# mwickert/scikit-dsp-comm

Measured on AMD Instinct MI355X. Metric: complex64 MSamples/s (FIR-1024 tap, 2^26 samples), higher is better.
Workload: dtype c64

## Files before the change

### scikit-dsp-comm_amd/csrc/fir_bank.hip

```cpp
#include "skdsp_internal.hpp"
#include "ols4k_tables.hpp"
#include "tile_walk.hpp"

namespace skdsp {

using namespace ols4k;
typedef float bank_v2f __attribute__((ext_vector_type(2)));

constexpr int64_t kBankTableCap = (int64_t)256 << 20;

struct FirBankHandle : HandleBase {
    int ntaps = 0, nbands = 0, ov = 0, V = 0;
    bool xr = false;
    DevTable<float2> tw, T2;
    DevTable<float4> Hp;
    DevTable<double> g64;
};

struct BankArgs {
    const void *x;
    cf *y;
    int64_t n, row_stride;
    const float2 *tw, *T2;
    const float4 *Hp;
// ... 65 lines not shown
        const float *x = reinterpret_cast<const float *>(A.x);
#pragma unroll 1
        for (int k = 0; k < c.ntaps && k <= m; ++k) {
            const double xv = (double)x[m - k];
            re += c.taps[2 * k] * xv;
            im += c.taps[2 * k + 1] * xv;
        }
    } else {
        careful_fir_point<float, true>(reinterpret_cast<const float *>(A.x), 0, c, 1, 1, m, &re, &im);
    }
    A.y[(size_t)band * A.row_stride + m] = make_float2((float)re, (float)im);
}

template <bool XR> __global__ __launch_bounds__(256, 2) void bank4k_kernel(BankArgs A)
{
    __shared__ cf img[kImgUnits];
    __shared__ cf T2f[kT2Units], T2t[kT2Units];
    __shared__ cf twl[kTwUnits];
    __shared__ unsigned long long noted_word;
    const int t = threadIdx.x;
    if (t == 0) noted_word = 0;
    walk::twiddles_4k(t, A.T2, A.tw, T2f, T2t, twl);
    __syncthreads();
    int64_t step = 0;
    for (int64_t item = blockIdx.x; item < A.items; item += gridDim.x, ++step) {
        const int group = (int)(item / A.ntiles);
        const int64_t tile = item - (int64_t)group * A.ntiles;
        const int b0 = group * A.per;
        const int b1 = b0 + A.per < A.nbands ? b0 + A.per : A.nbands;
        const int64_t out0 = tile * A.V;
        const int64_t in0 = out0 - A.ov;
        cf Z[16];
        float4 hh[8];
        bank_load_H(A, b0, t, hh);
        if (in0 >= 0 && in0 + kN <= A.n) {
            bank_load_interior<XR>(A, in0, t, Z);
        } else {
            bank_load_edge<XR>(A.x, in0, A.n, t, Z);
        }
        fwd_pass1(t, Z, twl, img);
        __syncthreads();
        fwd_pass2(t, T2f, img);
        fwd_pass3(t, img, Z);
        bool poisoned = false;
#pragma unroll 1
        for (int band = b0; band < b1; ++band) {
            cf P[16];
            mul_H(hh, Z, P);
            if (band + 1 < b1) bank_load_H(A, band + 1, t, hh);
            inv_pass3(t, T2t, img, P);
            inv_pass2(t, img);
            __syncthreads();
            inv_pass1(t, twl, img, P);
            __syncthreads();
            poisoned = poisoned || not_finite(P[15]);
            bank_store(A, band, out0, t, P);
        }
        if (__builtin_expect(__any(poisoned), 0)) careful_note(&noted_word, step);
    }
    const unsigned long long noted = careful_noted(&noted_word);
    if (__builtin_expect(noted != 0, 0)) {
        int64_t k = 0;
        for (int64_t item = blockIdx.x; item < A.items; item += gridDim.x, ++k) {
            if (!careful_step_noted(noted, k)) continue;
            const int group = (int)(item / A.ntiles);
            const int64_t out0 = (item - (int64_t)group * A.ntiles) * A.V;
            const int b0 = group * A.per;
            const int b1 = b0 + A.per < A.nbands ? b0 + A.per : A.nbands;
#pragma unroll 1
            for (int band = b0; band < b1; ++band)
#pragma unroll 1
                for (int i = t; i < A.V; i += 256) {
                    if (out0 + i >= A.n) break;
                    bank_careful_point<XR>(A, band, out0 + i);
                }
        }
    }
}

constexpr int kBankFwdCost = 3;
static int bank_bands_per_group(int64_t ntiles, int nbands, int64_t slots)
{
    int best = nbands;
    int64_t best_cost = INT64_MAX;
    for (int g = 1; g <= nbands; ++g) {
        const int per = (nbands + g - 1) / g;
        const int gg = (nbands + per - 1) / per;
// ... 84 lines not shown
```

### scikit-dsp-comm_amd/csrc/fir_dn4k.hip

```cpp
#include "skdsp_internal.hpp"
#include "ols4k_tables.hpp"
#include "tile_walk.hpp"

namespace skdsp {

using namespace ols4k;
typedef float v4f_t __attribute__((ext_vector_type(4)));
typedef float v2f_t __attribute__((ext_vector_type(2)));

struct Dn4kPlan : TilePlan {
    int ov = 0, V = 0;
    DevTable<float2> tw, T2;
    DevTable<float4> Hp;
};

struct Dn4kArgs {
    const void *x;
    void *y;
    int64_t n, n_hist;
    int64_t n_out;
    const float2 *tw, *T2;
    const float4 *Hp;
    int ov, V, a0;
    int M;
// ... 107 lines not shown
{
#pragma unroll 1
    for (int a = a0; a < 16; ++a) {
        const int64_t o = out0 + 256 * (a - a0) + t;
        if (REAL) {
            if (o < n_out) careful_fir_store<float, false>(reinterpret_cast<const float *>(x), n_hist, cf, 1, M, o, reinterpret_cast<float *>(y) + o);
            if (o + V < n_out) careful_fir_store<float, false>(reinterpret_cast<const float *>(x), n_hist, cf, 1, M, o + V, reinterpret_cast<float *>(y) + o + V);
        } else if (o < n_out) {
            careful_fir_store<float, true>(reinterpret_cast<const float *>(x), n_hist, cf, 1, M, o, reinterpret_cast<float *>(y) + 2 * o);
        }
    }
}

template <bool REAL, int MS> __global__ __launch_bounds__(256, 2) void dn4k_kernel(Dn4kArgs A)
{
    __shared__ cf img[kImgUnits];
    __shared__ cf T2f[kT2Units], T2t[kT2Units];
    __shared__ cf twl[kTwUnits];
    __shared__ unsigned long long dn_noted;
    const int t = threadIdx.x;
    if (t == 0) dn_noted = 0;
    walk::twiddles_4k(t, A.T2, A.tw, T2f, T2t, twl);
    __syncthreads();
    int64_t tile = walk::first_tile();
    cf in[MS * 16];
    bool have_in = false;
    for (; tile < A.ntiles; tile += gridDim.x) {
        const bool pre_next = tile + gridDim.x < A.ntiles && dn4k_interior<REAL>(A, tile + gridDim.x);
        if (!have_in) {
            if (dn4k_interior<REAL>(A, tile)) {
                dn4k_load_interior<REAL, MS>(A, tile, 0, t, in);
            } else {
                static_for<0, MS>([&](auto jc) __attribute__((always_inline)) {
                    constexpr int j = decltype(jc)::value;
                    cf e[16];
                    dn4k_load_edge<REAL>(A.x, dn4k_k0<REAL>(A, tile), A.V, A.M, j, A.n_hist, A.n, t, e);
#pragma unroll
                    for (int a = 0; a < 16; ++a) in[16 * j + a] = e[a];
                });
            }
        }
        have_in = pre_next;
        cf acc[16];
        static_for<0, MS>([&](auto jc) __attribute__((always_inline)) {
            constexpr int j = decltype(jc)::value;
            float4 hh[8];
            walk::load_H(A.Hp, j, t, hh);
            cf *Z = in + 16 * j;
            fwd_pass1(t, Z, twl, img);
            __syncthreads();
            fwd_pass2(t, T2f, img, Z);
            fwd_pass3(t, img, Z);
            walk::pin<16>(Z);
            if (j == 0) mul_H(hh, Z, acc); else mac_H(hh, Z, acc);
            walk::pin<16>(acc);
            __syncthreads();
        });
        if (pre_next) dn4k_load_interior<REAL, MS>(A, tile + gridDim.x, 0, t, in);
        inv_pass3(t, T2t, img, acc);
        inv_pass2(t, img);
        __syncthreads();
        inv_pass1(t, twl, img, acc);
        __syncthreads();
        walk::pin<16>(acc);
        if (pre_next) static_for<0, MS>([&](auto jc) __attribute__((always_inline)) { walk::pin<16>(in + 16 * decltype(jc)::value); });
        dn4k_store<REAL>(A, tile, t, acc);
        if (__builtin_expect(__any(not_finite(acc[15].x) | not_finite(acc[15].y)), 0)) careful_note(&dn_noted, (tile - walk::first_tile()) / gridDim.x);
    }
    const unsigned long long noted = careful_noted(&dn_noted);
    if (__builtin_expect(noted != 0, 0)) {
        int64_t k = 0;
        for (int64_t tl = walk::first_tile(); tl < A.ntiles; tl += gridDim.x, ++k)
            if (careful_step_noted(noted, k))
                dn4k_careful_outputs<REAL>(A.x, A.y, A.n_out, A.n_hist, A.cf, A.M, tl * (REAL ? 2 : 1) * (int64_t)A.V, A.V, A.a0, t);
    }
}

bool fir_dn4k_supported(const FirHandle *h, int M)
{
    if (M < 2 || M > 4) return false;
    const int T = dn_taps_per_phase(h->ntaps, M);
    if (T - 1 > 2048) return false;
    return h->dtype == SKDSP_C64 || (h->dtype == SKDSP_F32 && !h->taps_complex);
}

static int dn4k_plan(FirHandle *h, int M, Dn4kPlan **out)
{
    return tile_plan(h->dn4k, M, out, [&](Dn4kPlan &p) {
        tile_overlap(dn_taps_per_phase(h->ntaps, M), 256, kN, &p.ov, &p.V);
        std::vector<float2> tw, T2;
        std::vector<float4> Hp;
        make_tw(tw);
        make_T2(T2);
        make_dn_tables(h->taps_host.data(), h->ntaps, h->taps_complex ? 2 : 1, M, Hp);
        int rc = p.tw.upload(tw);
        if (!rc) rc = p.T2.upload(T2);
        if (!rc) rc = p.Hp.upload(Hp);
// ... 40 lines not shown
```

### scikit-dsp-comm_amd/csrc/fir_ols.hip

```cpp
#include "skdsp_internal.hpp"
#include "ols_tables.hpp"
#include <cstdlib>
#include <cstdio>


namespace skdsp {

using namespace ols;
typedef float v4f_t __attribute__((ext_vector_type(4)));

struct OlsPlan {
    int ntaps = 0;
    int ov = 0;
    int V = 0;
    float4 *T1 = nullptr, *T2 = nullptr, *Hp = nullptr;
};

struct OlsArgs {
    const cf *x;
    cf *y;
    int64_t n, n_hist;
    const float4 *T1, *T2, *Hp;
    int ov, V, a0;
    int keep;
// ... 104 lines not shown
        const int64_t q0 = out0 / A.dec;
        const unsigned r0 = (unsigned)(out0 - q0 * A.dec);
        const unsigned ob = r0 != 0 ? 1u : 0u;
        cf *buf = reinterpret_cast<cf *>(lds);
        int a0 = A.a0;
        asm volatile("" : "+s"(a0));
        __syncthreads();
#pragma unroll
        for (int a = 0; a < 16; ++a) {
            if (a < a0) continue;
#pragma unroll
            for (int e = 0; e < 2; ++e) {
                const unsigned gl = r0 + 512u * (unsigned)(a - a0) + 2u * (unsigned)t + (unsigned)e;
                const unsigned q = (unsigned)(((unsigned long long)gl * A.dec_magic) >> 32);
                if (q * M == gl) buf[q - ob] = v[2 * a + e];
            }
        }
        __syncthreads();
        int64_t oe = q0 + (int64_t)((r0 + (unsigned)A.V + M - 1) / M);
        const int64_t n_out = A.n_keep / A.dec;
        if (oe > n_out) oe = n_out;
        const int cnt = (int)(oe - (q0 + ob));
        cf *yo = A.y + q0 + ob;
        for (int i = t; i < cnt; i += 256) {
            const v2f_t o = {buf[i].x, buf[i].y};
            __builtin_nontemporal_store(o, reinterpret_cast<v2f_t *>(yo + i));
        }
        return;
    }
    if (full) {
        int tt = t;
        asm volatile("" : "+v"(tt));
        float4 *yp = reinterpret_cast<float4 *>(A.y + out0 + 2 * tt);
        auto stores = [&](auto a0c) __attribute__((always_inline)) {
            constexpr int A0 = decltype(a0c)::value;
#pragma unroll
            for (int a = A0; a < 16; ++a) {
                v4f_t nv;
                nv.x = v[2 * a].x; nv.y = v[2 * a].y; nv.z = v[2 * a + 1].x; nv.w = v[2 * a + 1].y;
                __builtin_nontemporal_store(nv, reinterpret_cast<v4f_t *>(yp) + (a - A0) * 256);
            }
        };
        switch (A.a0) {
            case 1: stores(std::integral_constant<int, 1>{}); break;
            case 2: stores(std::integral_constant<int, 2>{}); break;
            case 3: stores(std::integral_constant<int, 3>{}); break;
            case 4: stores(std::integral_constant<int, 4>{}); break;
// ... 286 lines not shown
{
    __shared__ float4 lds[kLdsUnits];
    __shared__ float4 t2lds[2 * kT2Units];
    __shared__ unsigned long long ols_noted;
    if (threadIdx.x == 0) ols_noted = 0;
    constexpr int HS = (DEC && !UP) ? (REAL ? 4 : 5) : 0;
    float4 *T2f = t2lds;
    float4 *T2t = t2lds + kT2Units;
    const int t = threadIdx.x;

    {
        const float4 w = A.T2[t];
        T2f[t] = w;
        T2t[(t & 15) * 16 + (t >> 4)] = w;
    }
    cf tw[16];
#pragma unroll
    for (int k1 = 1; k1 < 16; ++k1) tw[k1] = lo(A.T1[k1 * 256 + t]);
    tw[0] = make_float2(1.f, 0.f);

    __syncthreads();
    int it = 0;
    float4 hh[16];
    int64_t tile = (gridDim.x % 8 == 0) ? (int64_t)(blockIdx.x % 8) * (gridDim.x / 8) + blockIdx.x / 8
                                                                 : (int64_t)blockIdx.x;
    const bool t0_last = A.halo_flag != nullptr;
    auto phys = [&](int64_t w) -> int64_t {
        if (UP) return (int64_t)((unsigned)w / (unsigned)A.up);
        return t0_last ? (w + 1 < A.ntiles ? w + 1 : 0) : w;
    };
    auto phase_of = [&](int64_t w) -> int { return (int)((unsigned)w % (unsigned)A.up); };
    if (!UP) load_H(t, A.Hp, hh);
    cf v[32];
    if (tile < A.ntiles) {
        if (t0_last && phys(tile) == 0) wait_halo(A);
        load_any<REAL, XR>(A, phys(tile), t, v);
    }
    if constexpr (XR) {
#pragma unroll
        for (int i = 0; i < 32; i += 8)
            asm volatile("" ::"v"(v[i].x), "v"(v[i + 1].x), "v"(v[i + 2].x), "v"(v[i + 3].x), "v"(v[i + 4].x), "v"(v[i + 5].x), "v"(v[i + 6].x), "v"(v[i + 7].x));
    } else {
#pragma unroll
    for (int i = 0; i < 32; i += 8)
        asm volatile("" ::"v"(v[i].x), "v"(v[i].y), "v"(v[i + 1].x), "v"(v[i + 1].y), "v"(v[i + 2].x), "v"(v[i + 2].y),
                     "v"(v[i + 3].x), "v"(v[i + 3].y), "v"(v[i + 4].x), "v"(v[i + 4].y), "v"(v[i + 5].x), "v"(v[i + 5].y),
                     "v"(v[i + 6].x), "v"(v[i + 6].y), "v"(v[i + 7].x), "v"(v[i + 7].y));
    }
    for (; tile < A.ntiles; tile += gridDim.x, ++it) {
        if (HS > 0) {
            int tt = t;
            asm volatile("" : "+v"(tt));
#pragma unroll
            for (int j = 16 - HS; j < 16; ++j) hh[j] = vld(reinterpret_cast<const volatile float4 *>(A.Hp) + (unsigned)(j * 256 + tt));
        }
        if (UP) {
            int tt = t;
            asm volatile("" : "+v"(tt));
            const volatile float4 *hp = reinterpret_cast<const volatile float4 *>(A.Hp) + (size_t)phase_of(tile) * 4096;
#pragma unroll
            for (int j = 0; j < 16; ++j) hh[j] = vld(hp + (unsigned)(j * 256 + tt));
        }
        if (REAL) fwd_pass1_real(t, v, tw, lds); else fwd_pass1(t, v, tw, lds);
        __syncthreads();
        cf Z[32];
        fwd_pass23(t, T2f, lds, Z);
        mul_H(hh, Z);
        const int64_t next = tile + gridDim.x;
        cf nx[32];
        __builtin_amdgcn_s_setprio(3);
        if (next < A.ntiles) {
            if (t0_last && phys(next) == 0) wait_halo(A);
            load_any<REAL, XR>(A, phys(next), t, nx);
        }
        __builtin_amdgcn_s_setprio(0);
        inv_pass32(t, T2t, lds, Z);
        __syncthreads();
        inv_pass1(t, tw, lds, v);
        if constexpr (XR) {
#pragma unroll
            for (int i = 0; i < 32; i += 8)
                asm volatile("" ::"v"(nx[i].x), "v"(nx[i + 1].x), "v"(nx[i + 2].x), "v"(nx[i + 3].x), "v"(nx[i + 4].x), "v"(nx[i + 5].x), "v"(nx[i + 6].x), "v"(nx[i + 7].x)
                             : "memory");
        } else {
#pragma unroll
        for (int i = 0; i < 32; i += 8)
            asm volatile("" ::"v"(nx[i].x), "v"(nx[i].y), "v"(nx[i + 1].x), "v"(nx[i + 1].y), "v"(nx[i + 2].x), "v"(nx[i + 2].y),
                         "v"(nx[i + 3].x), "v"(nx[i + 3].y), "v"(nx[i + 4].x), "v"(nx[i + 4].y), "v"(nx[i + 5].x), "v"(nx[i + 5].y),
                         "v"(nx[i + 6].x), "v"(nx[i + 6].y), "v"(nx[i + 7].x), "v"(nx[i + 7].y)
                         : "memory");
        }
        __builtin_amdgcn_s_setprio(3);
        if (UP) {
            if (!DEC && A.up_pitch) {
                OlsArgs B = A;
                B.y = REAL ? reinterpret_cast<cf *>(reinterpret_cast<float *>(A.y) + (int64_t)phase_of(tile) * A.up_pitch) : A.y + (int64_t)phase_of(tile) * A.up_pitch;
                store_any<REAL, false>(B, phys(tile), t, v, lds);
            } else if (REAL) {
                store_tile_real_up<DEC>(A, phys(tile), phase_of(tile), t, v);
            } else {
                store_tile_up<DEC>(A, phys(tile), phase_of(tile), t, v);
            }
        } else {
            store_any<REAL, DEC>(A, phys(tile), t, v, lds);
        }
        __builtin_amdgcn_s_setprio(0);
        if (__builtin_expect(__any(not_finite(v[31].x) | not_finite(v[31].y)), 0)) careful_note(&ols_noted, it);
#pragma unroll
        for (int i = 0; i < 32; ++i) v[i] = nx[i];
#ifdef SK_OLS_KEEP_B3
        __syncthreads();
#else
        if constexpr (REAL || DEC || UP || XR) __syncthreads();
#endif
    }
    const unsigned long long noted = careful_noted(&ols_noted);
    if (__builtin_expect(noted != 0, 0)) {
        int64_t w = (gridDim.x % 8 == 0) ? (int64_t)(blockIdx.x % 8) * (gridDim.x / 8) + blockIdx.x / 8 : (int64_t)blockIdx.x;
        for (int64_t k = 0; w < A.ntiles; w += gridDim.x, ++k)
            if (careful_step_noted(noted, k))
                careful_ols_tile<float, REAL, DEC, UP, XR>(ols_careful_args(A, UP ? phase_of(w) : 0, !(REAL || XR)), phys(w), UP ? phase_of(w) : 0, t);
    }
}


template <bool REAL, int MF>
__global__ __launch_bounds__(256, 2) void ols_fold_kernel(OlsArgs A)
{
    __shared__ float4 lds[kLdsUnits];
    __shared__ float4 t2lds[2 * kT2Units];
    __shared__ unsigned long long ols_noted;
    if (threadIdx.x == 0) ols_noted = 0;
    float4 *T2f = t2lds, *T2t = t2lds + kT2Units;
    const int t = threadIdx.x;
    {
        const float4 w = A.T2[t];
        T2f[t] = w;
        T2t[(t & 15) * 16 + (t >> 4)] = w;
    }
    cf tw[16];
#pragma unroll
    for (int k1 = 1; k1 < 16; ++k1) tw[k1] = lo(A.T1[k1 * 256 + t]);
    tw[0] = make_float2(1.f, 0.f);
    __syncthreads();
    float4 hh[16];
    auto first_tile = [&]() -> int64_t { return (gridDim.x % 8 == 0) ? (int64_t)(blockIdx.x % 8) * (gridDim.x / 8) + blockIdx.x / 8 : (int64_t)blockIdx.x; };
    int64_t tile = first_tile();
    load_H(t, A.Hp, hh);
    cf v[32];
    if (tile < A.ntiles) load_any<REAL, false>(A, tile, t, v);
#pragma unroll
    for (int i = 0; i < 32; i += 8)
        asm volatile("" ::"v"(v[i].x), "v"(v[i].y), "v"(v[i + 1].x), "v"(v[i + 1].y), "v"(v[i + 2].x), "v"(v[i + 2].y),
                     "v"(v[i + 3].x), "v"(v[i + 3].y), "v"(v[i + 4].x), "v"(v[i + 4].y), "v"(v[i + 5].x), "v"(v[i + 5].y),
                     "v"(v[i + 6].x), "v"(v[i + 6].y), "v"(v[i + 7].x), "v"(v[i + 7].y));
    constexpr int LS = MF / 2;
    const int b = t >> 4, q = t & 15;
    const bool active = q % LS == 0;
    const int j0 = (32 / MF) * b + q / LS;
    constexpr int JA = 512 / MF;
    for (int64_t step = 0; tile < A.ntiles; tile += gridDim.x, ++step) {
        if (REAL) fwd_pass1_real(t, v, tw, lds); else fwd_pass1(t, v, tw, lds);
        __syncthreads();
        cf Z[32];
        fwd_pass23(t, T2f, lds, Z);
        mul_H(hh, Z);
        const int64_t next = tile + gridDim.x;
        cf nx[32];
        __builtin_amdgcn_s_setprio(3);
        if (next < A.ntiles) load_any<REAL, false>(A, next, t, nx);
        __builtin_amdgcn_s_setprio(0);
        inv_pass32_fold<MF>(t, T2t, lds, Z);
        __syncthreads();
        cf o[16];
#pragma unroll
        for (int a = 0; a < 16; ++a) o[a] = make_float2(0.f, 0.f);
        inv_pass1_fold<MF>(t, tw, lds, o);
#pragma unroll
        for (int i = 0; i < 32; i += 8)
            asm volatile("" ::"v"(nx[i].x), "v"(nx[i].y), "v"(nx[i + 1].x), "v"(nx[i + 1].y), "v"(nx[i + 2].x), "v"(nx[i + 2].y),
                         "v"(nx[i + 3].x), "v"(nx[i + 3].y), "v"(nx[i + 4].x), "v"(nx[i + 4].y), "v"(nx[i + 5].x), "v"(nx[i + 5].y),
                         "v"(nx[i + 6].x), "v"(nx[i + 6].y), "v"(nx[i + 7].x), "v"(nx[i + 7].y)
                         : "memory");
        __builtin_amdgcn_s_setprio(3);
        if (active) {
            int a0 = A.a0;
            asm volatile("" : "+s"(a0));
            const int Mr = A.dec / MF;
            const int64_t n_out = A.n_keep / A.dec;
            const int VD = A.V / MF;
            const int64_t e0 = (REAL ? 2 * tile : tile) * (int64_t)VD;
            const int64_t q0 = Mr > 1 ? e0 / Mr : e0;
            const unsigned r0 = Mr > 1 ? (unsigned)(e0 - q0 * Mr) : 0u;
// ... 7 lines not shown
                }
            };
#pragma unroll
            for (int a = 0; a < 16; ++a) {
                if (a < a0) continue;
                const unsigned el = (unsigned)(j0 + JA * (a - a0));
                if (REAL) {
                    put(el, o[a].x, reinterpret_cast<float *>(A.y));
                    put(el + (unsigned)VD, o[a].y, reinterpret_cast<float *>(A.y));
                } else {
                    put(el, v2f_t{o[a].x, o[a].y}, reinterpret_cast<v2f_t *>(A.y));
                }
            }
        }
        __builtin_amdgcn_s_setprio(0);
        if (__builtin_expect(__any(active && (not_finite(o[15].x) | not_finite(o[15].y))), 0)) careful_note(&ols_noted, step);
#pragma unroll
        for (int i = 0; i < 32; ++i) v[i] = nx[i];
#ifdef SK_OLS_KEEP_B3
        __syncthreads();
#else
        if constexpr (REAL) __syncthreads();
#endif
    }
    const unsigned long long noted = careful_noted(&ols_noted);
    if (__builtin_expect(noted != 0, 0)) {
        int64_t w = first_tile();
        for (int64_t k = 0; w < A.ntiles; w += gridDim.x, ++k)
            if (careful_step_noted(noted, k)) careful_ols_tile<float, REAL, true, false, false>(ols_careful_args(A, 0, !REAL), w, 0, t);
    }
}


template <bool REAL, int LF>
__device__ __forceinline__ void load_rep(const OlsArgs &A, int64_t tile, int t, cf *in)
{
    constexpr int LS = LF / 2, JA = 512 / LF;
    const int b = t >> 4, q = t & 15;
#pragma unroll
    for (int a = 0; a < 16; ++a) in[a] = make_float2(0.f, 0.f);
    if (q % LS != 0) return;
    const int j0 = (32 / LF) * b + q / LS;
    const int Lr = A.rep_lr;
    const int64_t in0 = (REAL ? 2 * tile : tile) * (int64_t)A.V - A.ov;
    const int64_t e0 = in0 / LF;
    int64_t q0 = e0, r0 = 0;
    if (Lr > 1) {
        q0 = e0 / Lr;
        r0 = e0 - q0 * Lr;
        if (r0 < 0) { r0 += Lr; q0 -= 1; }
    }
    const int VD = A.V / LF;
// ... 37 lines not shown
    }
}

template <bool REAL, int LF>
__global__ __launch_bounds__(256, 2) void ols_rep_kernel(OlsArgs A)
{
    __shared__ float4 lds[kLdsUnits];
    __shared__ float4 t2lds[2 * kT2Units];
    __shared__ unsigned long long ols_noted;
    if (threadIdx.x == 0) ols_noted = 0;
    float4 *T2f = t2lds, *T2t = t2lds + kT2Units;
    const int t = threadIdx.x;
    {
        const float4 w = A.T2[t];
        T2f[t] = w;
        T2t[(t & 15) * 16 + (t >> 4)] = w;
    }
    cf tw[16];
#pragma unroll
    for (int k1 = 1; k1 < 16; ++k1) tw[k1] = lo(A.T1[k1 * 256 + t]);
    tw[0] = make_float2(1.f, 0.f);
    __syncthreads();
    float4 hh[16];
    auto first_tile = [&]() -> int64_t { return (gridDim.x % 8 == 0) ? (int64_t)(blockIdx.x % 8) * (gridDim.x / 8) + blockIdx.x / 8 : (int64_t)blockIdx.x; };
    int64_t tile = first_tile();
    load_H(t, A.Hp, hh);
    cf in[16];
    if (tile < A.ntiles) load_rep<REAL, LF>(A, tile, t, in);
#pragma unroll
    for (int i = 0; i < 16; i += 8)
        asm volatile("" ::"v"(in[i].x), "v"(in[i].y), "v"(in[i + 1].x), "v"(in[i + 1].y), "v"(in[i + 2].x), "v"(in[i + 2].y),
                     "v"(in[i + 3].x), "v"(in[i + 3].y), "v"(in[i + 4].x), "v"(in[i + 4].y), "v"(in[i + 5].x), "v"(in[i + 5].y),
                     "v"(in[i + 6].x), "v"(in[i + 6].y), "v"(in[i + 7].x), "v"(in[i + 7].y));
    for (int64_t step = 0; tile < A.ntiles; tile += gridDim.x, ++step) {
        fwd_pass1_rep<LF>(t, in, tw, lds);
        __syncthreads();
        cf Z[32];
        fwd_pass23_rep<LF>(t, T2f, lds, Z);
        mul_H(hh, Z);
        const int64_t next = tile + gridDim.x;
        cf nx[16];
        __builtin_amdgcn_s_setprio(3);
        if (next < A.ntiles) load_rep<REAL, LF>(A, next, t, nx);
        __builtin_amdgcn_s_setprio(0);
        inv_pass32(t, T2t, lds, Z);
        __syncthreads();
        cf v[32];
        inv_pass1(t, tw, lds, v);
#pragma unroll
        for (int i = 0; i < 16; i += 8)
            asm volatile("" ::"v"(nx[i].x), "v"(nx[i].y), "v"(nx[i + 1].x), "v"(nx[i + 1].y), "v"(nx[i + 2].x), "v"(nx[i + 2].y),
                         "v"(nx[i + 3].x), "v"(nx[i + 3].y), "v"(nx[i + 4].x), "v"(nx[i + 4].y), "v"(nx[i + 5].x), "v"(nx[i + 5].y),
                         "v"(nx[i + 6].x), "v"(nx[i + 6].y), "v"(nx[i + 7].x), "v"(nx[i + 7].y)
                         : "memory");
        __builtin_amdgcn_s_setprio(3);
        store_any<REAL, false>(A, tile, t, v, lds);
        __builtin_amdgcn_s_setprio(0);
        if (__builtin_expect(__any(not_finite(v[31].x) | not_finite(v[31].y)), 0)) careful_note(&ols_noted, step);
#pragma unroll
        for (int i = 0; i < 16; ++i) in[i] = nx[i];
        __syncthreads();
    }
    const unsigned long long noted = careful_noted(&ols_noted);
    if (__builtin_expect(noted != 0, 0)) {
        int64_t w = first_tile();
        for (int64_t k = 0; w < A.ntiles; w += gridDim.x, ++k)
            if (careful_step_noted(noted, k))
                careful_fir_range<float, !REAL>(A.x, A.y, A.rep_hist, A.n, (REAL ? 2 * w : w) * (int64_t)A.V, (REAL ? 2 : 1) * (int64_t)A.V, A.rep_L, 1, A.cf, t);
    }
}

bool fir_ols_supported(const FirHandle *h)
{
    if (h->ntaps < 2 || h->ntaps - 1 > 4096) return false;
    return h->dtype == SKDSP_C64 || (h->dtype == SKDSP_F32 && !h->taps_complex);
}

static int build_plan(const FirHandle *h, int up, OlsPlan **out, int kind = 0)
{
    if (kind == 1) {
        const int T = (h->ntaps + up - 1) / up;
        OlsPlan *p = new OlsPlan();
        p->ntaps = T;
        p->ov = ((T - 1 + 511) / 512) * 512;
        if (p->ov == 0) p->ov = 512;
        p->V = kN - p->ov;
        std::vector<float4> T1, T2, Hp, Hall;
        make_T1(T1);
        make_T2(T2);
        std::vector<double> ph((size_t)T * 2);
// ... 315 lines not shown
```

### scikit-dsp-comm_amd/csrc/fir_up2k.hip

```cpp
#include "skdsp_internal.hpp"
#include "ols2k_tables.hpp"
#include "tile_walk.hpp"

namespace skdsp {

using namespace ols2k;
typedef float v4f_t __attribute__((ext_vector_type(4)));
typedef float v2f_t __attribute__((ext_vector_type(2)));

struct Up2kPlan : TilePlan {
    int ov = 0, V = 0, passes = 0;
    bool pairs = false;
    DevTable<float2> tw1, tw2, tw3;
    DevTable<float4> Hp;
};

struct Up2kArgs {
    const void *x;
    void *y;
    int64_t n, n_hist;
    const float2 *tw1, *tw2, *tw3;
    const float4 *Hp;
    int ov, V;
    int passes;
// ... 118 lines not shown
        const int s = 256 * m + t - ov;
        if (s < 0) continue;
        if (out0 + s >= n) break;
        careful_up_row<XR>(x, y, n_hist, cf, L, out0 + s);
    }
}

template <bool XR, int PH, bool STAGED> __global__ __launch_bounds__(256, 2) void up2k_kernel(Up2kArgs A)
{
    constexpr bool ZL = PH > 8;
    __shared__ cf img[kImgUnits];
    __shared__ cf tw1l[kTw1Units], tw2l[kTw2Units], tw3l[kTw3Units];
    __shared__ float4 stage[STAGED ? 4 * Up2kStage<PH>::kWaveUnits : 1];
    __shared__ cf zl[ZL ? 8 * 256 : 1];
    __shared__ unsigned long long up_noted;
    const int t = threadIdx.x;
    if (t == 0) up_noted = 0;
    {
        tw1l[t] = A.tw1[t]; tw1l[256 + t] = A.tw1[256 + t]; tw1l[512 + t] = A.tw1[512 + t];
        tw2l[t] = A.tw2[t]; tw2l[256 + t] = A.tw2[256 + t];
        if (t < kTw3Units) tw3l[t] = A.tw3[t];
    }
    __syncthreads();
    int64_t tile = walk::first_tile();
    cf Z[8];
    bool have_x = false;
    for (; tile < A.ntiles; tile += gridDim.x) {
        const bool has_next = tile + gridDim.x < A.ntiles;
        const bool pre_next = !ZL && has_next && up2k_interior(A, tile + gridDim.x);
        if (!have_x) {
            if (up2k_interior(A, tile)) {
                up2k_load_interior<XR>(A, tile, t, Z);
            } else {
                cf e[8];
                up2k_load_edge<XR>(A.x, tile * A.V - A.ov, A.n_hist, A.n, t, e);
#pragma unroll
                for (int m = 0; m < 8; ++m) Z[m] = e[m];
            }
        }
        have_x = pre_next;
        if constexpr (XR) {
#pragma unroll
            for (int m = 0; m < 8; ++m) Z[m].y = 0.f;
        }
        fwd_pass1(t, Z, tw1l, img);
        __syncthreads();
        fwd_pass2(t, tw2l, img);
        fwd_pass3(t, tw3l, img);
        fwd_pass4(t, img, Z);
        if constexpr (ZL) {
#pragma unroll
            for (int k = 0; k < 8; ++k) zl[k * 256 + t] = Z[k];
// ... 1 lines not shown
        bool poisoned = false;
        for (int g0 = 0; g0 < A.passes; g0 += PH) {
            const int cnt = A.passes - g0 < PH ? A.passes - g0 : PH;
            const bool last_group = g0 + cnt == A.passes;
            cf out[PH * 8];
            static_for<0, PH>([&](auto qc) __attribute__((always_inline)) {
                constexpr int q = decltype(qc)::value;
                if (q < cnt) {
                    float4 hh[4];
                    {
                        int tt = t;
                        asm volatile("" : "+v"(tt));
                        const volatile float4 *hp = reinterpret_cast<const volatile float4 *>(A.Hp) + (size_t)(g0 + q) * 1024;
#pragma unroll
                        for (int k = 0; k < 4; ++k) hh[k] = walk::vld(hp + (unsigned)(k * 256 + tt));
                    }
                    if constexpr (ZL) {
#pragma unroll
                        for (int k = 0; k < 8; ++k) out[8 * q + k] = zl[k * 256 + t];
                        mul_H(hh, out + 8 * q, out + 8 * q);
                    } else {
                        mul_H(hh, Z, out + 8 * q);
                        if (q == cnt - 1 && last_group && pre_next)
                            up2k_load_interior<XR>(A, tile + gridDim.x, t, Z);
                    }
                    inv_pass4(t, img, out + 8 * q);
                    inv_pass3<ZL>(t, tw3l, img);
                    inv_pass2<ZL>(t, tw2l, img);
                    __syncthreads();
                    inv_pass1(t, tw1l, img, out + 8 * q);
                    __syncthreads();
                    walk::pin<8>(out + 8 * q);
                }
            });
            if (!ZL && last_group && pre_next) walk::settle_x<XR, 8>(Z);
            poisoned |= not_finite(out[7].x) | not_finite(out[7].y);
            if constexpr (STAGED) {
                up2k_store_staged<PH>(A, tile, cnt, t, out, stage + Up2kStage<PH>::kWaveUnits * (t >> 6));
            } else if constexpr (XR) {
                if (A.odd_tail && last_group) up2k_store_direct<PH, true>(A, tile, g0, cnt, t, out);
                else up2k_store_direct<PH, false>(A, tile, g0, cnt, t, out);
            } else {
                up2k_store_direct<PH, false>(A, tile, g0, cnt, t, out);
            }
        }
        if (__builtin_expect(__any(poisoned), 0)) careful_note(&up_noted, (tile - walk::first_tile()) / gridDim.x);
    }
    const unsigned long long noted = careful_noted(&up_noted);
    if (__builtin_expect(noted != 0, 0)) {
        int64_t k = 0;
        for (int64_t tl = walk::first_tile(); tl < A.ntiles; tl += gridDim.x, ++k)
            if (careful_step_noted(noted, k)) up2k_careful_rows<XR>(A.x, A.y, A.n, A.n_hist, A.cf, A.row_bytes / (XR ? 4 : 8), tl * A.V, A.ov, t);
    }
}

bool fir_up2k_supported(const FirHandle *h, int L)
{
    if (L < 2 || L > 256) return false;
    const int T = up_taps_per_phase(h->ntaps, L);
    if (T - 1 > 1024) return false;
    return h->dtype == SKDSP_C64 || (h->dtype == SKDSP_F32 && !h->taps_complex);
}

static int up2k_plan(FirHandle *h, int L, Up2kPlan **out)
{
    return tile_plan(h->up2k, L, out, [&](Up2kPlan &p) {
        p.pairs = h->dtype == SKDSP_F32;
        tile_overlap(up_taps_per_phase(h->ntaps, L), 64, k2N, &p.ov, &p.V);
        p.passes = up_passes(L, p.pairs);
        std::vector<float2> tw1, tw2, tw3;
        std::vector<float4> Hp;
        make_tw1(tw1);
        make_tw2(tw2);
        make_tw3(tw3);
        make_up_tables(h->taps_host.data(), h->ntaps, h->taps_complex ? 2 : 1, L, p.pairs, Hp);
// ... 55 lines not shown
```

### scikit-dsp-comm_amd/csrc/fir_up4k.hip

```cpp
#include "skdsp_internal.hpp"
#include "ols4k_tables.hpp"
#include "tile_walk.hpp"

namespace skdsp {

using namespace ols4k;
typedef float v4f_t __attribute__((ext_vector_type(4)));
typedef float v2f_t __attribute__((ext_vector_type(2)));

struct Up4kPlan : TilePlan {
    int ov = 0, V = 0, passes = 0;
    bool pairs = false;
    DevTable<float2> tw, T2;
    DevTable<float4> Hp;
};

struct Up4kArgs {
    const void *x;
    void *y;
    int64_t n, n_hist;
    const float2 *tw, *T2;
    const float4 *Hp;
    int ov, V, a0;
    int passes;
// ... 122 lines not shown
    for (int k = 0; k < 8; ++k) hh[k] = make_float4(0.f, 0.f, 0.f, 0.f);
}
template <bool XR> __device__ __forceinline__ void up4k_careful_rows(const void *x, void *y, int64_t n, int64_t n_hist, const CarefulFir cf, int L, int64_t out0, int a0, int t)
{
#pragma unroll 1
    for (int a = a0; a < 16; ++a) {
        const int64_t i = out0 + 256 * (a - a0) + t;
        if (i >= n) break;
        careful_up_row<XR>(x, y, n_hist, cf, L, i);
    }
}

template <bool XR, int G> __global__ __launch_bounds__(256, 2) void up4k_kernel(Up4kArgs A)
{
    __shared__ cf img[kImgUnits];
    __shared__ cf T2f[kT2Units], T2t[kT2Units];
    __shared__ cf twl[kTwUnits];
    __shared__ float4 stage[G == 4 ? 4 * 128 : 1];
    __shared__ unsigned long long up_noted;
    const int t = threadIdx.x;
    if (t == 0) up_noted = 0;
    walk::twiddles_4k(t, A.T2, A.tw, T2f, T2t, twl);
    __syncthreads();
    int64_t tile = walk::first_tile();
    cf Z[16];
    float4 hh[G][8];
    bool have_x = false;
    if (tile < A.ntiles) {
        walk::load_H(A.Hp, 0, t, hh[0]);
    } else {
        up4k_no_H(hh[0]);
    }
    for (; tile < A.ntiles; tile += gridDim.x) {
        const bool has_next = tile + gridDim.x < A.ntiles;
        const bool pre_next = has_next && up4k_interior(A, tile + gridDim.x);
        if (!have_x) {
            if (up4k_interior(A, tile)) {
                up4k_load_interior<XR>(A, tile, t, Z);
            } else {
                cf e[16];
                up4k_load_edge<XR>(A.x, tile * A.V - A.ov, A.n_hist, A.n, t, e);
#pragma unroll
                for (int a = 0; a < 16; ++a) Z[a] = e[a];
            }
        }
        have_x = pre_next;
        if constexpr (XR) {
#pragma unroll
            for (int a = 0; a < 16; ++a) Z[a].y = 0.f;
        }
        fwd_pass1(t, Z, twl, img);
        __syncthreads();
        fwd_pass2(t, T2f, img);
        fwd_pass3(t, img, Z);
        bool poisoned = false;
        for (int g0 = 0; g0 < A.passes; g0 += G) {
            const int cnt = A.passes - g0 < G ? A.passes - g0 : G;
            const bool last_group = g0 + cnt == A.passes;
            cf out[G * 16];
            static_for<0, G>([&](auto jc) __attribute__((always_inline)) {
                constexpr int j = decltype(jc)::value;
                if (j < cnt) {
                    cf P[16];
                    if (j > 0) walk::load_H(A.Hp, g0 + j, t, hh[j]);
                    mul_H(hh[j], Z, P);
                    if (j == cnt - 1 && last_group && pre_next)
                        up4k_load_interior<XR>(A, tile + gridDim.x, t, Z);
                    inv_pass3(t, T2t, img, P);
                    inv_pass2(t, img);
                    __syncthreads();
                    inv_pass1(t, twl, img, out + 16 * j);
                    __syncthreads();
                    walk::pin<16>(out + 16 * j);
                }
            });
            if (!last_group) walk::load_H(A.Hp, g0 + G, t, hh[0]);
            else if (has_next) walk::load_H(A.Hp, 0, t, hh[0]);
            else up4k_no_H(hh[0]);
            walk::settle<8>(hh[0]);
            if (last_group && pre_next) walk::settle_x<XR, 16>(Z);
            poisoned |= not_finite(out[15].x) | not_finite(out[15].y);
            const bool tail = A.odd_tail && last_group;
            auto store = [&](auto tc) __attribute__((always_inline)) {
                constexpr bool TAIL = decltype(tc)::value;
                if constexpr (G == 4) {
                    if (cnt == 4) {
                        if (!TAIL && A.staged) up4k_store4_staged(A, tile, g0, t, out, stage + 128 * (t >> 6));
                        else up4k_store<4, TAIL>(A, tile, g0, t, out);
                        return;
                    }
                    if (cnt == 3) { up4k_store<3, TAIL>(A, tile, g0, t, out); return; }
                }
                if (cnt == 2) up4k_store<2, TAIL>(A, tile, g0, t, out);
                else up4k_store<1, TAIL>(A, tile, g0, t, out);
            };
            if constexpr (XR) {
                if (tail) store(std::true_type{}); else store(std::false_type{});
            } else {
                store(std::false_type{});
            }
        }
        if (__builtin_expect(__any(poisoned), 0)) careful_note(&up_noted, (tile - walk::first_tile()) / gridDim.x);
    }
    const unsigned long long noted = careful_noted(&up_noted);
    if (__builtin_expect(noted != 0, 0)) {
        int64_t k = 0;
        for (int64_t tl = walk::first_tile(); tl < A.ntiles; tl += gridDim.x, ++k)
            if (careful_step_noted(noted, k)) up4k_careful_rows<XR>(A.x, A.y, A.n, A.n_hist, A.cf, A.row_bytes / (XR ? 4 : 8), tl * A.V, A.a0, t);
    }
}

bool fir_up4k_supported(const FirHandle *h, int L)
{
    if (L < 2 || L > 256) return false;
    const int T = up_taps_per_phase(h->ntaps, L);
    if (T - 1 > 2048) return false;
    return h->dtype == SKDSP_C64 || (h->dtype == SKDSP_F32 && !h->taps_complex);
}

static int up4k_plan(FirHandle *h, int L, Up4kPlan **out)
{
    return tile_plan(h->up4k, L, out, [&](Up4kPlan &p) {
        p.pairs = h->dtype == SKDSP_F32;
        tile_overlap(up_taps_per_phase(h->ntaps, L), 256, kN, &p.ov, &p.V);
        p.passes = up_passes(L, p.pairs);
        std::vector<float2> tw, T2;
        std::vector<float4> Hp;
        make_tw(tw);
        make_T2(T2);
        make_up_tables(h->taps_host.data(), h->ntaps, h->taps_complex ? 2 : 1, L, p.pairs, Hp);
        int rc = p.tw.upload(tw);
// ... 42 lines not shown
```

### scikit-dsp-comm_amd/csrc/tile_walk.hpp

```cpp
#pragma once
#include "ols_core.hpp"

namespace skdsp {
namespace walk {

using ols::cf;

__device__ __forceinline__ int64_t first_tile()
{
    return (gridDim.x % 8 == 0) ? (int64_t)(blockIdx.x % 8) * (gridDim.x / 8) + blockIdx.x / 8 : (int64_t)blockIdx.x;
}

__device__ __forceinline__ void twiddles_4k(int t, const float2 *T2, const float2 *tw, cf *T2f, cf *T2t, cf *twl)
{
    const cf w = T2[t];
    T2f[t] = w;
    T2t[(t & 15) * 16 + (t >> 4)] = w;
#pragma unroll
    for (int k = 0; k < 15; ++k) twl[k * 256 + t] = tw[k * 256 + t];
}

__device__ __forceinline__ float4 vld(const volatile float4 *p)
{
    float4 r;
    r.x = p->x; r.y = p->y; r.z = p->z; r.w = p->w;
    return r;
}
__device__ __forceinline__ void load_H(const float4 *Hp, int q, int t, float4 *hh)
{
    int tt = t;
    asm volatile("" : "+v"(tt));
    const volatile float4 *hp = reinterpret_cast<const volatile float4 *>(Hp) + (size_t)q * 2048;
#pragma unroll
// ... 10 lines not shown
template <int N> __device__ __forceinline__ void settle(const float4 *hh)
{
#pragma unroll
    for (int k = 0; k < N; k += 4)
        asm volatile("" ::"v"(hh[k].x), "v"(hh[k].y), "v"(hh[k].z), "v"(hh[k].w), "v"(hh[k + 1].x), "v"(hh[k + 1].y), "v"(hh[k + 1].z), "v"(hh[k + 1].w),
                     "v"(hh[k + 2].x), "v"(hh[k + 2].y), "v"(hh[k + 2].z), "v"(hh[k + 2].w), "v"(hh[k + 3].x), "v"(hh[k + 3].y), "v"(hh[k + 3].z), "v"(hh[k + 3].w)
                     : "memory");
}
template <bool XR, int N> __device__ __forceinline__ void settle_x(const cf *v)
{
    if constexpr (XR) {
#pragma unroll
        for (int i = 0; i < N; i += 8)
            asm volatile("" ::"v"(v[i].x), "v"(v[i + 1].x), "v"(v[i + 2].x), "v"(v[i + 3].x), "v"(v[i + 4].x), "v"(v[i + 5].x), "v"(v[i + 6].x), "v"(v[i + 7].x) : "memory");
    } else {
#pragma unroll
        for (int i = 0; i < N; i += 8)
            asm volatile("" ::"v"(v[i].x), "v"(v[i].y), "v"(v[i + 1].x), "v"(v[i + 1].y), "v"(v[i + 2].x), "v"(v[i + 2].y), "v"(v[i + 3].x), "v"(v[i + 3].y),
                         "v"(v[i + 4].x), "v"(v[i + 4].y), "v"(v[i + 5].x), "v"(v[i + 5].y), "v"(v[i + 6].x), "v"(v[i + 6].y), "v"(v[i + 7].x), "v"(v[i + 7].y)
                         : "memory");
    }
}

}
}
```

Measured before the change: 296,200.

## Redistribute tail tiles across XCD-interleaved blocks with precomputed tile walk

Replaces the grid-stride tile loop in all OLS/bank/up/down kernels with a precomputed Tiles walker. It handles the full rounds as before, then spreads the partial last round evenly across the 8 XCD groups, optionally aligning to the upsampling phase unit. Loops now run a fixed step count with int counters instead of comparing against ntiles each time. This aims to balance the final partial wave across chiplets, at the cost of more complex index arithmetic and a shifted last-tile mapping.

```diff
diff --git a/scikit-dsp-comm_amd/csrc/fir_bank.hip b/scikit-dsp-comm_amd/csrc/fir_bank.hip
--- a/scikit-dsp-comm_amd/csrc/fir_bank.hip
+++ b/scikit-dsp-comm_amd/csrc/fir_bank.hip
@@ -111,8 +111,9 @@
     if (t == 0) noted_word = 0;
     walk::twiddles_4k(t, A.T2, A.tw, T2f, T2t, twl);
     __syncthreads();
-    int64_t step = 0;
-    for (int64_t item = blockIdx.x; item < A.items; item += gridDim.x, ++step) {
+    const walk::Tiles W = walk::tiles(A.items);
+    int64_t item = W.first;
+    for (int step = 0; step < W.steps; item = W.next(item, step), ++step) {
         const int group = (int)(item / A.ntiles);
         const int64_t tile = item - (int64_t)group * A.ntiles;
         const int b0 = group * A.per;
@@ -149,9 +150,10 @@
     }
     const unsigned long long noted = careful_noted(&noted_word);
     if (__builtin_expect(noted != 0, 0)) {
-        int64_t k = 0;
-        for (int64_t item = blockIdx.x; item < A.items; item += gridDim.x, ++k) {
+        const walk::Tiles Wr = walk::tiles_again(A.items);
+        for (int k = 0; k < Wr.steps; ++k) {
             if (!careful_step_noted(noted, k)) continue;
+            const int64_t item = Wr.at(k);
             const int group = (int)(item / A.ntiles);
             const int64_t out0 = (item - (int64_t)group * A.ntiles) * A.V;
             const int b0 = group * A.per;
diff --git a/scikit-dsp-comm_amd/csrc/fir_dn4k.hip b/scikit-dsp-comm_amd/csrc/fir_dn4k.hip
--- a/scikit-dsp-comm_amd/csrc/fir_dn4k.hip
+++ b/scikit-dsp-comm_amd/csrc/fir_dn4k.hip
@@ -153,11 +153,13 @@
     if (t == 0) dn_noted = 0;
     walk::twiddles_4k(t, A.T2, A.tw, T2f, T2t, twl);
     __syncthreads();
-    int64_t tile = walk::first_tile();
+    const walk::Tiles W = walk::tiles(A.ntiles);
+    int64_t tile = W.first;
     cf in[MS * 16];
     bool have_in = false;
-    for (; tile < A.ntiles; tile += gridDim.x) {
-        const bool pre_next = tile + gridDim.x < A.ntiles && dn4k_interior<REAL>(A, tile + gridDim.x);
+    for (int step = 0; step < W.steps; ++step) {
+        const int64_t next = W.next(tile, step);
+        const bool pre_next = step + 1 < W.steps && dn4k_interior<REAL>(A, next);
         if (!have_in) {
             if (dn4k_interior<REAL>(A, tile)) {
                 dn4k_load_interior<REAL, MS>(A, tile, 0, t, in);
@@ -187,7 +189,7 @@
             walk::pin<16>(acc);
             __syncthreads();
         });
-        if (pre_next) dn4k_load_interior<REAL, MS>(A, tile + gridDim.x, 0, t, in);
+        if (pre_next) dn4k_load_interior<REAL, MS>(A, next, 0, t, in);
         inv_pass3(t, T2t, img, acc);
         inv_pass2(t, img);
         __syncthreads();
@@ -196,14 +198,15 @@
         walk::pin<16>(acc);
         if (pre_next) static_for<0, MS>([&](auto jc) __attribute__((always_inline)) { walk::pin<16>(in + 16 * decltype(jc)::value); });
         dn4k_store<REAL>(A, tile, t, acc);
-        if (__builtin_expect(__any(not_finite(acc[15].x) | not_finite(acc[15].y)), 0)) careful_note(&dn_noted, (tile - walk::first_tile()) / gridDim.x);
+        if (__builtin_expect(__any(not_finite(acc[15].x) | not_finite(acc[15].y)), 0)) careful_note(&dn_noted, step);
+        tile = next;
     }
     const unsigned long long noted = careful_noted(&dn_noted);
     if (__builtin_expect(noted != 0, 0)) {
-        int64_t k = 0;
-        for (int64_t tl = walk::first_tile(); tl < A.ntiles; tl += gridDim.x, ++k)
+        const walk::Tiles Wr = walk::tiles_again(A.ntiles);
+        for (int k = 0; k < Wr.steps; ++k)
             if (careful_step_noted(noted, k))
-                dn4k_careful_outputs<REAL>(A.x, A.y, A.n_out, A.n_hist, A.cf, A.M, tl * (REAL ? 2 : 1) * (int64_t)A.V, A.V, A.a0, t);
+                dn4k_careful_outputs<REAL>(A.x, A.y, A.n_out, A.n_hist, A.cf, A.M, Wr.at(k) * (REAL ? 2 : 1) * (int64_t)A.V, A.V, A.a0, t);
     }
 }
 
diff --git a/scikit-dsp-comm_amd/csrc/fir_ols.hip b/scikit-dsp-comm_amd/csrc/fir_ols.hip
--- a/scikit-dsp-comm_amd/csrc/fir_ols.hip
+++ b/scikit-dsp-comm_amd/csrc/fir_ols.hip
@@ -1,5 +1,6 @@
 #include "skdsp_internal.hpp"
 #include "ols_tables.hpp"
+#include "tile_walk.hpp"
 #include <cstdlib>
 #include <cstdio>
 
@@ -150,7 +151,9 @@
         if (oe > n_out) oe = n_out;
         const int cnt = (int)(oe - (q0 + ob));
         cf *yo = A.y + q0 + ob;
-        for (int i = t; i < cnt; i += 256) {
+        int tt = t;
+        asm volatile("" : "+v"(tt));
+        for (int i = tt; i < cnt; i += 256) {
             const v2f_t o = {buf[i].x, buf[i].y};
             __builtin_nontemporal_store(o, reinterpret_cast<v2f_t *>(yo + i));
         }
@@ -483,8 +486,8 @@
     __syncthreads();
     int it = 0;
     float4 hh[16];
-    int64_t tile = (gridDim.x % 8 == 0) ? (int64_t)(blockIdx.x % 8) * (gridDim.x / 8) + blockIdx.x / 8
-                                                                 : (int64_t)blockIdx.x;
+    const walk::Tiles W = walk::tiles(A.ntiles, UP ? (unsigned)A.up : 1u);
+    int64_t tile = W.first;
     const bool t0_last = A.halo_flag != nullptr;
     auto phys = [&](int64_t w) -> int64_t {
         if (UP) return (int64_t)((unsigned)w / (unsigned)A.up);
@@ -493,7 +496,7 @@
     auto phase_of = [&](int64_t w) -> int { return (int)((unsigned)w % (unsigned)A.up); };
     if (!UP) load_H(t, A.Hp, hh);
     cf v[32];
-    if (tile < A.ntiles) {
+    if (W.steps > 0) {
         if (t0_last && phys(tile) == 0) wait_halo(A);
         load_any<REAL, XR>(A, phys(tile), t, v);
     }
@@ -508,7 +511,7 @@
                      "v"(v[i + 3].x), "v"(v[i + 3].y), "v"(v[i + 4].x), "v"(v[i + 4].y), "v"(v[i + 5].x), "v"(v[i + 5].y),
                      "v"(v[i + 6].x), "v"(v[i + 6].y), "v"(v[i + 7].x), "v"(v[i + 7].y));
     }
-    for (; tile < A.ntiles; tile += gridDim.x, ++it) {
+    for (; it < W.steps; ++it) {
         if (HS > 0) {
             int tt = t;
             asm volatile("" : "+v"(tt));
@@ -527,10 +530,10 @@
         cf Z[32];
         fwd_pass23(t, T2f, lds, Z);
         mul_H(hh, Z);
-        const int64_t next = tile + gridDim.x;
+        const int64_t next = W.next(tile, it);
         cf nx[32];
         __builtin_amdgcn_s_setprio(3);
-        if (next < A.ntiles) {
+        if (it + 1 < W.steps) {
             if (t0_last && phys(next) == 0) wait_halo(A);
             load_any<REAL, XR>(A, phys(next), t, nx);
         }
@@ -574,12 +577,13 @@
 #else
         if constexpr (REAL || DEC || UP || XR) __syncthreads();
 #endif
+        tile = next;
     }
     const unsigned long long noted = careful_noted(&ols_noted);
     if (__builtin_expect(noted != 0, 0)) {
-        int64_t w = (gridDim.x % 8 == 0) ? (int64_t)(blockIdx.x % 8) * (gridDim.x / 8) + blockIdx.x / 8 : (int64_t)blockIdx.x;
-        for (int64_t k = 0; w < A.ntiles; w += gridDim.x, ++k)
-            if (careful_step_noted(noted, k))
+        const walk::Tiles Wr = walk::tiles_again(A.ntiles, UP ? (unsigned)A.up : 1u);
+        for (int k = 0; k < Wr.steps; ++k)
+            if (int64_t w = Wr.at(k); careful_step_noted(noted, k))
                 careful_ols_tile<float, REAL, DEC, UP, XR>(ols_careful_args(A, UP ? phase_of(w) : 0, !(REAL || XR)), phys(w), UP ? phase_of(w) : 0, t);
     }
 }
@@ -605,11 +609,11 @@
     tw[0] = make_float2(1.f, 0.f);
     __syncthreads();
     float4 hh[16];
-    auto first_tile = [&]() -> int64_t { return (gridDim.x % 8 == 0) ? (int64_t)(blockIdx.x % 8) * (gridDim.x / 8) + blockIdx.x / 8 : (int64_t)blockIdx.x; };
-    int64_t tile = first_tile();
+    const walk::Tiles W = walk::tiles(A.ntiles);
+    int64_t tile = W.first;
     load_H(t, A.Hp, hh);
     cf v[32];
-    if (tile < A.ntiles) load_any<REAL, false>(A, tile, t, v);
+    if (W.steps > 0) load_any<REAL, false>(A, tile, t, v);
 #pragma unroll
     for (int i = 0; i < 32; i += 8)
         asm volatile("" ::"v"(v[i].x), "v"(v[i].y), "v"(v[i + 1].x), "v"(v[i + 1].y), "v"(v[i + 2].x), "v"(v[i + 2].y),
@@ -620,16 +624,16 @@
     const bool active = q % LS == 0;
     const int j0 = (32 / MF) * b + q / LS;
     constexpr int JA = 512 / MF;
-    for (int64_t step = 0; tile < A.ntiles; tile += gridDim.x, ++step) {
+    for (int step = 0; step < W.steps; ++step) {
         if (REAL) fwd_pass1_real(t, v, tw, lds); else fwd_pass1(t, v, tw, lds);
         __syncthreads();
         cf Z[32];
         fwd_pass23(t, T2f, lds, Z);
         mul_H(hh, Z);
-        const int64_t next = tile + gridDim.x;
+        const int64_t next = W.next(tile, step);
         cf nx[32];
         __builtin_amdgcn_s_setprio(3);
-        if (next < A.ntiles) load_any<REAL, false>(A, next, t, nx);
+        if (step + 1 < W.steps) load_any<REAL, false>(A, next, t, nx);
         __builtin_amdgcn_s_setprio(0);
         inv_pass32_fold<MF>(t, T2t, lds, Z);
         __syncthreads();
@@ -683,12 +687,13 @@
 #else
         if constexpr (REAL) __syncthreads();
 #endif
+        tile = next;
     }
     const unsigned long long noted = careful_noted(&ols_noted);
     if (__builtin_expect(noted != 0, 0)) {
-        int64_t w = first_tile();
-        for (int64_t k = 0; w < A.ntiles; w += gridDim.x, ++k)
-            if (careful_step_noted(noted, k)) careful_ols_tile<float, REAL, true, false, false>(ols_careful_args(A, 0, !REAL), w, 0, t);
+        const walk::Tiles Wr = walk::tiles_again(A.ntiles);
+        for (int k = 0; k < Wr.steps; ++k)
+            if (careful_step_noted(noted, k)) careful_ols_tile<float, REAL, true, false, false>(ols_careful_args(A, 0, !REAL), Wr.at(k), 0, t);
     }
 }
 
@@ -772,26 +777,26 @@
     tw[0] = make_float2(1.f, 0.f);
     __syncthreads();
     float4 hh[16];
-    auto first_tile = [&]() -> int64_t { return (gridDim.x % 8 == 0) ? (int64_t)(blockIdx.x % 8) * (gridDim.x / 8) + blockIdx.x / 8 : (int64_t)blockIdx.x; };
-    int64_t tile = first_tile();
+    const walk::Tiles W = walk::tiles(A.ntiles);
+    int64_t tile = W.first;
     load_H(t, A.Hp, hh);
     cf in[16];
-    if (tile < A.ntiles) load_rep<REAL, LF>(A, tile, t, in);
+    if (W.steps > 0) load_rep<REAL, LF>(A, tile, t, in);
 #pragma unroll
     for (int i = 0; i < 16; i += 8)
         asm volatile("" ::"v"(in[i].x), "v"(in[i].y), "v"(in[i + 1].x), "v"(in[i + 1].y), "v"(in[i + 2].x), "v"(in[i + 2].y),
                      "v"(in[i + 3].x), "v"(in[i + 3].y), "v"(in[i + 4].x), "v"(in[i + 4].y), "v"(in[i + 5].x), "v"(in[i + 5].y),
                      "v"(in[i + 6].x), "v"(in[i + 6].y), "v"(in[i + 7].x), "v"(in[i + 7].y));
-    for (int64_t step = 0; tile < A.ntiles; tile += gridDim.x, ++step) {
+    for (int step = 0; step < W.steps; ++step) {
         fwd_pass1_rep<LF>(t, in, tw, lds);
         __syncthreads();
         cf Z[32];
         fwd_pass23_rep<LF>(t, T2f, lds, Z);
         mul_H(hh, Z);
-        const int64_t next = tile + gridDim.x;
+        const int64_t next = W.next(tile, step);
         cf nx[16];
         __builtin_amdgcn_s_setprio(3);
-        if (next < A.ntiles) load_rep<REAL, LF>(A, next, t, nx);
+        if (step + 1 < W.steps) load_rep<REAL, LF>(A, next, t, nx);
         __builtin_amdgcn_s_setprio(0);
         inv_pass32(t, T2t, lds, Z);
         __syncthreads();
@@ -810,12 +815,13 @@
 #pragma unroll
         for (int i = 0; i < 16; ++i) in[i] = nx[i];
         __syncthreads();
+        tile = next;
     }
     const unsigned long long noted = careful_noted(&ols_noted);
     if (__builtin_expect(noted != 0, 0)) {
-        int64_t w = first_tile();
-        for (int64_t k = 0; w < A.ntiles; w += gridDim.x, ++k)
-            if (careful_step_noted(noted, k))
+        const walk::Tiles Wr = walk::tiles_again(A.ntiles);
+        for (int k = 0; k < Wr.steps; ++k)
+            if (int64_t w = Wr.at(k); careful_step_noted(noted, k))
                 careful_fir_range<float, !REAL>(A.x, A.y, A.rep_hist, A.n, (REAL ? 2 * w : w) * (int64_t)A.V, (REAL ? 2 : 1) * (int64_t)A.V, A.rep_L, 1, A.cf, t);
     }
 }
diff --git a/scikit-dsp-comm_amd/csrc/fir_up2k.hip b/scikit-dsp-comm_amd/csrc/fir_up2k.hip
--- a/scikit-dsp-comm_amd/csrc/fir_up2k.hip
+++ b/scikit-dsp-comm_amd/csrc/fir_up2k.hip
@@ -164,12 +164,14 @@
         if (t < kTw3Units) tw3l[t] = A.tw3[t];
     }
     __syncthreads();
-    int64_t tile = walk::first_tile();
+    const walk::Tiles W = walk::tiles(A.ntiles);
+    int64_t tile = W.first;
     cf Z[8];
     bool have_x = false;
-    for (; tile < A.ntiles; tile += gridDim.x) {
-        const bool has_next = tile + gridDim.x < A.ntiles;
-        const bool pre_next = !ZL && has_next && up2k_interior(A, tile + gridDim.x);
+    for (int step = 0; step < W.steps; ++step) {
+        const bool has_next = step + 1 < W.steps;
+        const int64_t next = W.next(tile, step);
+        const bool pre_next = !ZL && has_next && up2k_interior(A, next);
         if (!have_x) {
             if (up2k_interior(A, tile)) {
                 up2k_load_interior<XR>(A, tile, t, Z);
@@ -217,7 +219,7 @@
                     } else {
                         mul_H(hh, Z, out + 8 * q);
                         if (q == cnt - 1 && last_group && pre_next)
-                            up2k_load_interior<XR>(A, tile + gridDim.x, t, Z);
+                            up2k_load_interior<XR>(A, next, t, Z);
                     }
                     inv_pass4(t, img, out + 8 * q);
                     inv_pass3<ZL>(t, tw3l, img);
@@ -239,13 +241,14 @@
                 up2k_store_direct<PH, false>(A, tile, g0, cnt, t, out);
             }
         }
-        if (__builtin_expect(__any(poisoned), 0)) careful_note(&up_noted, (tile - walk::first_tile()) / gridDim.x);
+        if (__builtin_expect(__any(poisoned), 0)) careful_note(&up_noted, step);
+        tile = next;
     }
     const unsigned long long noted = careful_noted(&up_noted);
     if (__builtin_expect(noted != 0, 0)) {
-        int64_t k = 0;
-        for (int64_t tl = walk::first_tile(); tl < A.ntiles; tl += gridDim.x, ++k)
-            if (careful_step_noted(noted, k)) up2k_careful_rows<XR>(A.x, A.y, A.n, A.n_hist, A.cf, A.row_bytes / (XR ? 4 : 8), tl * A.V, A.ov, t);
+        const walk::Tiles Wr = walk::tiles_again(A.ntiles);
+        for (int k = 0; k < Wr.steps; ++k)
+            if (careful_step_noted(noted, k)) up2k_careful_rows<XR>(A.x, A.y, A.n, A.n_hist, A.cf, A.row_bytes / (XR ? 4 : 8), Wr.at(k) * A.V, A.ov, t);
     }
 }
 
diff --git a/scikit-dsp-comm_amd/csrc/fir_up4k.hip b/scikit-dsp-comm_amd/csrc/fir_up4k.hip
--- a/scikit-dsp-comm_amd/csrc/fir_up4k.hip
+++ b/scikit-dsp-comm_amd/csrc/fir_up4k.hip
@@ -168,18 +168,20 @@
     if (t == 0) up_noted = 0;
     walk::twiddles_4k(t, A.T2, A.tw, T2f, T2t, twl);
     __syncthreads();
-    int64_t tile = walk::first_tile();
+    const walk::Tiles W = walk::tiles(A.ntiles);
+    int64_t tile = W.first;
     cf Z[16];
     float4 hh[G][8];
     bool have_x = false;
-    if (tile < A.ntiles) {
+    if (W.steps > 0) {
         walk::load_H(A.Hp, 0, t, hh[0]);
     } else {
         up4k_no_H(hh[0]);
     }
-    for (; tile < A.ntiles; tile += gridDim.x) {
-        const bool has_next = tile + gridDim.x < A.ntiles;
-        const bool pre_next = has_next && up4k_interior(A, tile + gridDim.x);
+    for (int step = 0; step < W.steps; ++step) {
+        const bool has_next = step + 1 < W.steps;
+        const int64_t next = W.next(tile, step);
+        const bool pre_next = has_next && up4k_interior(A, next);
         if (!have_x) {
             if (up4k_interior(A, tile)) {
                 up4k_load_interior<XR>(A, tile, t, Z);
@@ -211,7 +213,7 @@
                     if (j > 0) walk::load_H(A.Hp, g0 + j, t, hh[j]);
                     mul_H(hh[j], Z, P);
                     if (j == cnt - 1 && last_group && pre_next)
-                        up4k_load_interior<XR>(A, tile + gridDim.x, t, Z);
+                        up4k_load_interior<XR>(A, next, t, Z);
                     inv_pass3(t, T2t, img, P);
                     inv_pass2(t, img);
                     __syncthreads();
@@ -246,13 +248,14 @@
                 store(std::false_type{});
             }
         }
-        if (__builtin_expect(__any(poisoned), 0)) careful_note(&up_noted, (tile - walk::first_tile()) / gridDim.x);
+        if (__builtin_expect(__any(poisoned), 0)) careful_note(&up_noted, step);
+        tile = next;
     }
     const unsigned long long noted = careful_noted(&up_noted);
     if (__builtin_expect(noted != 0, 0)) {
-        int64_t k = 0;
-        for (int64_t tl = walk::first_tile(); tl < A.ntiles; tl += gridDim.x, ++k)
-            if (careful_step_noted(noted, k)) up4k_careful_rows<XR>(A.x, A.y, A.n, A.n_hist, A.cf, A.row_bytes / (XR ? 4 : 8), tl * A.V, A.a0, t);
+        const walk::Tiles Wr = walk::tiles_again(A.ntiles);
+        for (int k = 0; k < Wr.steps; ++k)
+            if (careful_step_noted(noted, k)) up4k_careful_rows<XR>(A.x, A.y, A.n, A.n_hist, A.cf, A.row_bytes / (XR ? 4 : 8), Wr.at(k) * A.V, A.a0, t);
     }
 }
 
diff --git a/scikit-dsp-comm_amd/csrc/tile_walk.hpp b/scikit-dsp-comm_amd/csrc/tile_walk.hpp
--- a/scikit-dsp-comm_amd/csrc/tile_walk.hpp
+++ b/scikit-dsp-comm_amd/csrc/tile_walk.hpp
@@ -1,4 +1,5 @@
 #pragma once
+#include <stdint.h>
 #include "ols_core.hpp"
 
 namespace skdsp {
@@ -6,9 +7,68 @@
 
 using ols::cf;
 
-__device__ __forceinline__ int64_t first_tile()
+constexpr int64_t kNoTile = INT64_MAX;
+
+struct Tiles {
+    int64_t first;
+    unsigned G;
+    unsigned delta;
+    int steps;
+    SK_HD int64_t at(int k) const
+    {
+        if (k >= steps) return kNoTile;
+        return k == 0 ? first : first + (int64_t)(k < steps - 1 ? k : steps - 2) * G + (k < steps - 1 ? 0u : delta);
+    }
+    SK_HD int64_t next(int64_t tile, int k) const { return tile + (k + 2 == steps ? delta : G); }
+};
+
+SK_HD int64_t div_tiles(int64_t a, unsigned b) { return (a >> 32) == 0 ? (int64_t)((unsigned)a / b) : a / (int64_t)b; }
+
+SK_HD Tiles tiles_of(unsigned b, unsigned G, int64_t ntiles, unsigned unit = 1)
 {
-    return (gridDim.x % 8 == 0) ? (int64_t)(blockIdx.x % 8) * (gridDim.x / 8) + blockIdx.x / 8 : (int64_t)blockIdx.x;
+    Tiles w;
+    w.G = G;
+    const int nfull = (int)div_tiles(ntiles, G);
+    const int64_t base = (int64_t)nfull * G;
+    const unsigned R = (unsigned)(ntiles - base);
+    unsigned first = b, last = G;
+    if (G % 8 != 0) {
+        if (b < R) last = b;
+    } else {
+        const unsigned S = G / 8, x = b % 8;
+#ifdef SK_WALK_TAIL_HIGH_SLOTS
+        const unsigned j = S - 1 - b / 8;
+#else
+        const unsigned j = b / 8;
+#endif
+        first = x * S + b / 8;
+        const unsigned q = R / 8, r = R % 8;
+        unsigned lo = x * q + (x < r ? x : r), hi = (x + 1) * q + (x + 1 < r ? x + 1 : r);
+        if (unit > 1 && q + (r != 0) + unit - 1 <= S) {
+            const unsigned phase = (unsigned)(base - div_tiles(base, unit) * unit);
+            auto down = [&](unsigned s) -> unsigned {
+                if (s == 0 || s == R) return s;
+                const unsigned m = (phase + s) % unit;
+                return s > m ? s - m : 0;
+            };
+            lo = down(lo);
+            hi = down(hi);
+        }
+        if (j < hi - lo) last = lo + j;
+    }
+    w.steps = nfull + (last != G);
+    w.first = nfull ? (int64_t)first : (int64_t)last;
+    w.delta = last != G ? G + last - first : G;
+    return w;
+}
+
+#if defined(__HIPCC__)
+__device__ __forceinline__ Tiles tiles(int64_t ntiles, unsigned unit = 1) { return tiles_of(blockIdx.x, gridDim.x, ntiles, unit); }
+__device__ __forceinline__ Tiles tiles_again(int64_t ntiles, unsigned unit = 1)
+{
+    unsigned b = blockIdx.x;
+    asm volatile("" : "+s"(b));
+    return tiles_of(b, gridDim.x, ntiles, unit);
 }
 
 __device__ __forceinline__ void twiddles_4k(int t, const float2 *T2, const float2 *tw, cf *T2f, cf *T2t, cf *twl)
@@ -65,5 +125,7 @@
     }
 }
 
+#endif
+
 }
 }
```

Result: no change. 294,500 (median of 3 runs) (-0.6%).
